# winddori2002/DEX-TTS

Hardware: AMD Instinct MI355X
Metric: mel-frames/s at n_timesteps=50, 80-ch mel (sampler only); RTF (higher is better)
Workload: dtype bf16; 1 GPU; gedex_b1: gedex_lj B=1/GPU T=512 n_timesteps=50 (BASELINE.json configs[1]); global_batch=1, frames=512, hipgraph=False, parallelism=1 GPU

## Files before the change

dex_tts_amd/csrc/dex_api.hip:

```cpp
#include <hip/hip_runtime.h>
#include <cstdlib>

#include <cmath>
#include <cstdarg>
#include <atomic>
#include <cstdio>
#include <mutex>
#include <cstring>
#include <map>
#include <unordered_map>
#include <string_view>
#include <string>
#include <vector>

#include "../../include/dex_amd.h"
#include "kernels.h"
#include "weight_store.h"

using namespace dex;

namespace dex {
namespace {
const char* const KNOB_NAMES[] = {
    "DEX_CONV_STREAM", "DEX_CONV_PP", "DEX_CONV_SKIP_DEAD", "DEX_H_BF16", "DEX_ATTN_SEPARATE", "DEX_ATTN_Q64", "DEX_ATTN_Q64_TAIL", "DEX_ATTN_Q64_HALF", "DEX_DIT_XCDS", "DEX_ATTN_GENERIC", "DEX_RES2", "DEX_LP_INTER", "DEX_DIT_CHAIN",
    "DEX_DIT_CLUSTER", "DEX_DIT_CLUSTER_LOCAL", "DEX_ATTN_X_LP", "DEX_RES_X_LP", "DEX_CAT_LP", "DEX_XCD_MAP", "DEX_DEBUG_DROP_HANDOFF", "DEX_PATCH_FUSED",
    "DEX_CONV_DOWN", "DEX_CONVT_UP", "DEX_DEBUG_PLAN",
    "DEX_ATTN_SHARED_W8", "DEX_CONVT_MT", "DEX_CONVT_WGS", "DEX_CONV_DOWN_WGS", "DEX_CONV_REGW", "DEX_CONV_REGW_RES", "DEX_CONV_SMALL_MAX", "DEX_CONV_TH8",
    "DEX_CONV_W8", "DEX_DWCONV_CAP", "DEX_FINAL_CAP", "DEX_FIRST_CAP", "DEX_FIRST_MFMA", "DEX_GEMM_NWALK", "DEX_NWALK_SPLIT", "DEX_NWALK_BM", "DEX_POS_COL", "DEX_POS_COL_MIN",
    "DEX_POS_CT", "DEX_REGW_MIN_TILES", "DEX_REGW_WGS", "DEX_ROWCHAIN64", "DEX_ROWCHAIN64A", "DEX_TIV_CAP", "DEX_TV_CHAIN", "DEX_TIV_FOLD", "DEX_LINATTN_NSUB", "DEX_TV_FOLD", "DEX_OUT2_MIN", "DEX_NWALK_DMA",
    "DEX_LINATTN_HEADWAVES"};
constexpr int N_KNOBS = (int)(sizeof(KNOB_NAMES) / sizeof(KNOB_NAMES[0]));
int knob_parse(const char* e) {
    if (!e) return KNOB_UNSET;
    char* end = nullptr;
    const long v = strtol(e, &end, 10);
    if (end == e) {
        static bool warned = false;
        if (!warned) { warned = true; fprintf(stderr, "libdexamd: ignoring a DEX_* knob whose value '%s' is not an integer\n", e); }
        return KNOB_UNSET;
    }
    return (int)v;
}
struct KnobSnapshot {
    int v[N_KNOBS];
    KnobSnapshot() { for (int i = 0; i < N_KNOBS; ++i) v[i] = knob_parse(getenv(KNOB_NAMES[i])); }
};
thread_local const KnobSnapshot* t_knobs = nullptr;
struct WsplitScope {
    bool prev;
    explicit WsplitScope(bool on) : prev(g_lp_wsplit) { g_lp_wsplit = on; }
    ~WsplitScope() { g_lp_wsplit = prev; }
};
struct KnobScope {
    const KnobSnapshot* prev;
    explicit KnobScope(const KnobSnapshot* k) : prev(t_knobs) { t_knobs = k; }
    ~KnobScope() { t_knobs = prev; }
};
}
static int knob_index(const char* name) {
    static const std::unordered_map<std::string_view, int> idx = [] {
        std::unordered_map<std::string_view, int> m;
        for (int i = 0; i < N_KNOBS; ++i) m.emplace(KNOB_NAMES[i], i);
        return m;
    }();
    const auto it = idx.find(std::string_view(name));
    return it == idx.end() ? -1 : it->second;
}
int knob(const char* name) {
    if (t_knobs) {
        const int i = knob_index(name);
        if (i >= 0) return t_knobs->v[i];
    }
    return knob_parse(getenv(name));
}
}
static_assert(PREC_FP32 == DEX_PREC_FP32 && PREC_BF16 == DEX_PREC_BF16 && PREC_FP16 == DEX_PREC_FP16 && PREC_FP16X2 == DEX_PREC_FP16X2, "kernels.h mirrors DexPrecision");

namespace {
void xcd_map_probe();

struct TD { float* p; int ld; int coff; int C; int lp = 0; };

struct ResW { const float *w1, *b1, *g1, *be1, *w2, *b2, *g2, *be2, *wr, *br, *mlp_w, *mlp_b; int cin, cout; };
// ... 865 lines not shown
    }

    bool lp_inter_cur = false;
    bool cat_lp = false;
    IGemmP final_gemm(int mask_ws, float* out, int ldo, int ocoff) {
        const DexConfig& c = x->cfg;
        const int hid = c.dit_hidden, mid = mid_dim(c);
        const bool fuse_lnf = x->lp() && ln_fusable(hid);
        const int s2c = c.dit_stride * c.dit_stride * mid;
        IGemmP fl = base_gemm(fuse_lnf ? P.tok : P.xn, hid, 0, P.Hf, P.Wt, hid, x->fl_w, s2c, x->fl_b, out, ldo, ocoff);
        if (fuse_lnf) { fl.ln_shift = P.fin_mod; fl.ln_scale = P.fin_mod + hid; fl.ln_step_stride = 2L * hid; }
        { auto it = x->frag_of().find(x->fl_w); fl.Wfrag = (it != x->frag_of().end()) ? it->second : nullptr; }
        fl.unpatch_s = c.dit_stride; fl.unpatch_C = mid; fl.OHf = P.Hm; fl.OWf = P.Wm;
        fl.c_bstride = (long)P.Hm * P.Wm * ldo;
        fl.outmask = mask; fl.outmask_ws = mask_ws;
        return fl;
    }
    bool linattn_fused(int C) const { return x->lp() && (C == 64 || C == 128) && linattn_fused_supported(C); }
    void linattn(const LinW& w, const StageBuf& s, const TD& X, float* out, int ldo, int ocoff, const LinKvCtxP* tail = nullptr, bool out_lp = false,
                 void* out2_lp = nullptr, int ldo2 = 0, int ocoff2 = 0) {
        const long npix = s.npix; const int B = P.d.B;
        if (linattn_fused(X.C)) {
            int nsub = 1;
            while (nsub < 4 && (npix + 128 * nsub - 1) / (128 * nsub) * B > 192) nsub *= 2;
            {
                const int ncu = device_cus();
                const long slots = (long)(X.C == 64 ? 2 : 1) * ncu;
                if ((npix + 127) / 128 * B >= 2 * slots) {
                    long best = -1;
                    for (int n = 1; n <= 8; ++n) {
                        const long wgs = (npix + 128L * n - 1) / (128L * n) * B;
                        const long cost = (wgs + slots - 1) / slots * n;
                        if (best < 0 || cost <= best) { best = cost; nsub = n; }
                    }
                }
                const int forced = knob_or("DEX_LINATTN_NSUB", 0);
                if (forced > 0) nsub = forced;
            }
            const int nblk = (int)((npix + 128L * nsub - 1) / (128L * nsub));
            LinKvCtxP k{};
            if (tail) k = *tail;
            k.X = X.p; k.ldx = X.ld; k.x_coff = X.coff; k.xb = npix * X.ld; k.npix = (int)npix; k.C = X.C; k.Wkv = w.wkv_lp[x->lpi()];
            k.wkv_lo_off = x->lpi() == 2 ? 384L * X.C : 0;
            k.nsub = nsub; k.nblk = nblk; k.part_m = s.pm; k.part_s = s.ps; k.part_c = s.pc; k.B = B;
            k.headwaves = knob_or("DEX_LINATTN_HEADWAVES", (long)nblk * B <= device_cus() ? 1 : 0) != 0 ? 1 : 0;
            const bool xlp = k.H2 && k.Xout && lp_inter_cur && linattn_out2_lp_out_supported((int)npix, B) && !knob_off("DEX_ATTN_X_LP");
            k.xout_lp = xlp ? 1 : 0;
            run("linattn_kvctx", 2.0 * npix * B * (256.0 * X.C + 128 * 32), (tail ? (tail->h2_bf16 ? 10.0 : 12.0) - (xlp ? 2.0 : 0.0) : 4.0) * npix * X.C * B, [&] { launch_linattn_kvctx(k, x->precision, st); });
            LinMergeP mg{s.pm, s.ps, s.pc, nblk, w.wout_raw, w.g, X.C, s.mbf, B};
            run("linattn_merge", 2.0 * 128 * 32 * X.C * B, 4.0 * nblk * 4 * 1088 * B, [&] { launch_linattn_merge(mg, x->precision, st); });
            LinOut2P o{X.p, X.ld, X.coff, npix * X.ld, (int)npix, X.C, w.wq_frag[x->lpi()], s.mbf, w.bias_eff, out, ldo, ocoff, npix * ldo, B, out_lp ? 1 : 0,
                       out2_lp, ldo2, ocoff2, npix * ldo2, xlp ? 1 : 0};
            o.wq_lo_off = x->lpi() == 2 ? 128L * X.C : 0;
            run("linattn_out", 4.0 * npix * B * 128.0 * X.C, ((out_lp ? 6.0 : 8.0) - (xlp ? 2.0 : 0.0) + (out2_lp ? 2.0 : 0.0)) * npix * X.C * B, [&] { launch_linattn_out2(o, x->precision, st); });
            return;
        }
        IGemmP g = base_gemm(X.p, X.ld, X.coff, s.H, s.W, X.C, w.wqkv, 384, nullptr, s.qkv, 384, 0);
        gemm("linattn_qkv", g);
        LinAttnCtxP cp{s.qkv, 384, npix * 384, (int)npix, 4, LA_CHUNK, s.nchunks, s.pm, s.ps, s.pc, B};
        run("linattn_ctx", 2.0 * npix * 128 * 32 * B, 4.0 * npix * 384 * B, [&] { launch_linattn_ctx(cp, st); });
        LinAttnCombineP cb{s.pm, s.ps, s.pc, s.nchunks, 4, w.wout_raw, w.g, w.C, s.weff, B};
        run("linattn_combine", 2.0 * 128 * 32 * w.C * B, 4.0 * s.nchunks * 4 * 1100 * B, [&] { launch_linattn_combine(cb, st); });
        IGemmP o = base_gemm(s.qkv, 384, 0, s.H, s.W, 128, s.weff, w.C, w.bias_eff, out, ldo, ocoff);
        o.w_bstride = 128L * w.C;
        o.res = X.p; o.ldres = X.ld; o.res_coff = X.coff; o.res_bstride = npix * X.ld;
        gemm("linattn_out", o);
    }

    void dit(const TD& X, bool mask_input, int mask_ws, float* out, int ldo, int ocoff, const float* in_aff = nullptr) {
        const DexConfig& c = x->cfg;
        const int B = P.d.B, hid = c.dit_hidden, mid = mid_dim(c), N = P.N, mh = mlp_hidden(c);
        DwConvP dw{};
        dw.X = X.p + X.coff; dw.ldx = X.ld; dw.xb = (long)P.Hm * P.Wm * X.ld; dw.Hi = P.Hm; dw.Wi = P.Wm; dw.C = mid;
        dw.k = c.dit_patch; dw.s = c.dit_stride; dw.pad = c.dit_patch / 2; dw.Wd = x->pe_dw; dw.bd = x->pe_db;
        dw.mask = mask_input ? mask : nullptr; dw.mask_ws = mask_ws; dw.mask_bstride = P.d.T;
        dw.Y = P.pe0; dw.Hf = P.Hf; dw.Wt = P.Wt; dw.B = B; dw.aff = in_aff;
        auto pw_lp = x->lp_of().find(x->pe_pw);
        if (patch_fused()) {
            run("patch_embed", 2.0 * B * N * mid * (c.dit_patch * c.dit_patch + hid), 4.0 * B * (P.Hm * P.Wm * mid + N * hid),
                [&] { launch_patch_embed_fused(dw, pw_lp->second, x->pe_pb, P.emb, hid, x->precision, st); });
        } else {
            run("patch_dwconv_silu", 2.0 * B * N * mid * c.dit_patch * c.dit_patch, 4.0 * B * (P.Hm * P.Wm + N) * mid, [&] { launch_dwconv_silu(dw, st); });
            IGemmP pe = base_gemm(P.pe0, mid, 0, P.Hf, P.Wt, mid, x->pe_pw, hid, x->pe_pb, P.emb, hid, 0);
            gemm("patch_pointwise", pe);
        }
        const int G = c.dit_conv_pos_groups, kp = c.dit_conv_pos, cg = hid / G;
        int nsplit = POS_SPLIT, pcg = 0, pcgp = 0;
        if (x->lp() && x->pos_wfrag[x->lpi()]) {
            PosConvP pcd{P.emb, x->pos_wfrag[x->lpi()], P.pos_part, P.Hf, P.Wt, hid, G, B};
            run("pos_conv", 2.0 * B * N * (double)kp * kp * cg * hid, 8.0 * B * N * hid + 2.0 * kp * kp * cg * hid, [&] { launch_pos_conv_direct(pcd, x->precision, st); });
            nsplit = 1;
        } else {
            const int cgp = (cg % 32) ? 64 : cg;
            const float* src = P.emb;
            if (cgp != cg) {
                run("pos_group_pad", 0, 8.0 * B * N * hid, [&] { launch_group_pad(P.emb, P.emb_pad, (long)B * N, G, cg, cgp, st); });
                src = P.emb_pad;
            }
            IGemmP pc = base_gemm(src, G * cgp, 0, P.Hf, P.Wt, cgp, x->pos_w, cgp, nullptr, P.pos_part, G * cgp, 0);
            pc.KH = kp; pc.KW = kp; pc.off_h = -(kp / 2); pc.off_w = -(kp / 2); pc.K = kp * kp * cgp;
            pc.groups = G; pc.w_gstride = (long)kp * kp * cgp * cgp; pc.ksplit = POS_SPLIT; pc.c_sstride = (long)B * N * G * cgp;
            if (cgp != cg) pc.Wbf = nullptr;
            gemm("pos_conv", pc);
            pcg = cgp != cg ? cg : 0; pcgp = cgp;
        }
        PosFinishP pf{P.pos_part, nsplit, (long)B * N * (pcg ? G * pcgp : hid), x->pos_b, P.emb, x->freq_pos, P.tok, P.Hf, P.Wt, hid, B, pcg, pcgp};
// ... 813 lines not shown
```

dex_tts_amd/csrc/kernels.h:

```cpp
#pragma once
#include <hip/hip_runtime.h>
#include <stdint.h>

namespace dex {

constexpr int KNOB_UNSET = -2147483647 - 1;
int knob(const char* name);
inline int knob_or(const char* name, int dflt) { const int v = knob(name); return v == KNOB_UNSET ? dflt : v; }
inline bool knob_off(const char* name) { return knob(name) == 0; }
inline bool knob_set(const char* name) { return knob(name) != KNOB_UNSET; }
inline int device_cus() {
    static const int n = [] { int dev = 0, v = 0; (void)hipGetDevice(&dev); (void)hipDeviceGetAttribute(&v, hipDeviceAttributeMultiprocessorCount, dev); return v > 0 ? v : 256; }();
    return n;
}

constexpr int GN_SLOTS = 32;
typedef long long gnfix_t;

extern thread_local const char* g_last_symbol;

constexpr int PREC_FP32 = 0, PREC_BF16 = 1, PREC_FP16 = 2, PREC_FP16X2 = 3;
inline bool prec_wsplit(int precision) { return precision == PREC_FP16X2; }
extern thread_local bool g_lp_wsplit;
inline bool prec_is_lp(int precision) { return precision != PREC_FP32; }
// ... 98 lines not shown
};
void launch_gn_apply(const GnApplyP& p, hipStream_t st);

struct FinalP {
    const float* X; long xb; int npix, W, C, groups; const gnfix_t* stats; const float* gamma; const float* beta;
    const float* mask; long mask_bstride;
    const float* wfc; const float* bfc;
    const float* xcur;
    float* denoised;
    float* xnext;
    const float* scal; int scal_stride; int step;
    float* zero_ptr; long zero_n;
    int B;
    int mode; const float* htab; float* dbuf; const float* xhat;
    int x_bf16;
    const int* poison;
};
void launch_final(const FinalP& p, hipStream_t st);
void launch_churn_tables(const float* sigmas, int n, float S_churn, float S_min, float S_max, float S_noise,
                         float* t_hat, float* h, float* ncoef, hipStream_t st);
void launch_add_noise(float* x, const float* noise, const float* ncoef_i, long n, hipStream_t st);
void launch_heun_expand(const float* t_hat, const float* h, int n, float* sig, float* hout, hipStream_t st);

struct LinAttnCtxP { const float* qkv; int ld; long bstride; int n; int heads; int chunk; int nchunks;
                     float* part_m; float* part_s; float* part_c; int B; };
void launch_linattn_ctx(const LinAttnCtxP& p, hipStream_t st);
struct LinAttnCombineP { const float* part_m; const float* part_s; const float* part_c; int nchunks; int heads;
                         const float* Wout;
                         const float* g;
                         int C; float* Weff;
                         int B; };
void launch_linattn_combine(const LinAttnCombineP& p, hipStream_t st);

struct LinKvCtxP { const float* X; int ldx; int x_coff; long xb; int npix; int C; const void* Wkv; int nsub; int nblk;
                   float* part_m; float* part_s; float* part_c; int B;
                   const float* H2; const gnfix_t* gn_stats; const float* gamma; const float* beta;
                   const float* res; int ldres; long resb; int res_under_mask;
                   const float* mask; int mask_ws; long mask_bstride; int W; float* Xout;
                   int h2_bf16;
                   int res_lp;
                   int xout_lp;     long wkv_lo_off = 0;
                   int headwaves = 0;
                   long long* dbg = nullptr;
};
void launch_linattn_kvctx(const LinKvCtxP& p, int precision, hipStream_t st);
struct LinMergeP { const float* part_m; const float* part_s; const float* part_c; int nblk;
                   const float* Wout; const float* g; int C; void* W2; int B; };
void launch_linattn_merge(const LinMergeP& p, int precision, hipStream_t st);
struct LinOut2P { const float* X; int ldx; int x_coff; long xb; int npix; int C; const void* Wq; const void* W2;
                  const float* bias; float* Y; int ldy; int y_coff; long yb; int B;
                  int y_lp;
                  void* Y2; int ldy2; int y2_coff; long y2b;
                  int x_lp;     long wq_lo_off = 0;
                  };
void launch_linattn_out2(const LinOut2P& p, int precision, hipStream_t st);
bool linattn_out2_lp_out_supported(int npix, int B);
bool linattn_fused_supported(int C);

struct DwConvP { const float* X; int ldx; long xb; int Hi, Wi, C; int k, s, pad; const float* Wd; const float* bd;
                 const float* mask; int mask_ws; long mask_bstride;
                 float* Y; int Hf, Wt; int B;
                 const float* aff = nullptr; };
void launch_dwconv_silu(const DwConvP& p, hipStream_t st);
bool patch_embed_fused_supported(int k, int C, int hid, long ntok);
void launch_patch_embed_fused(const DwConvP& p, const void* Wb, const float* bias, float* emb, int hid, int precision, hipStream_t st);

struct PosConvP { const float* X; const void* Wf; float* Y; int Hf, Wt, hid, G, B;
                  int ncol; };
bool pos_conv_direct_supported(int hid, int groups, int kernel, int Hf);
void launch_pos_conv_direct(const PosConvP& p, int precision, hipStream_t st);
struct PosFinishP { const float* part; int nsplit; long split_stride; const float* bias; const float* emb;
                    const float* freq_pos; float* tok; int Hf, Wt, D; int B;
                    int cg, cg_pad; };
void launch_pos_finish(const PosFinishP& p, hipStream_t st);
void launch_group_pad(const float* src, float* dst, long rows, int G, int cg, int cg_pad, hipStream_t st);

struct LnModP { const float* X; float* Y; int rows_per_batch; int D; const float* shift; const float* scale;
                long step_stride; int step; int B; };
void launch_ln_mod(const LnModP& p, hipStream_t st);

struct DitChainP { const float* O; int ksplit; long o_sstride; const float* ml; int heads; int rows_per_batch;
                   float* X; const void *Wp, *W1, *W2, *Wq; const float *bp, *b1, *b2, *bq;
                   const float* ada;
                   const float *next_shift, *next_scale; long next_step_stride;
                   void *Qh, *Kh, *Vt; int Npad; float qscale;
                   const void *Qin, *Kin, *Vin;
                   int qkv_only;
                   int attn_inline;
                   int step; int M; int B; long long* dbg;
                   float* xslab; unsigned* xflag; unsigned epoch; int* xerr;
                   int o_lp;
                   int xcd_map;
                   int xlocal;
                   int xdrop;
                   int tail_row0 = 0, tail_ks = 0;
                   int xcds = 8; };
constexpr int DIT_CLUSTER = 4;
constexpr size_t DIT_CLUSTER_SLAB_FLOATS = 2 * DIT_CLUSTER * (32 * 256 + 256);
constexpr size_t DIT_CLUSTER_FLAG_WORDS = 2 * DIT_CLUSTER;
bool dit_rowchain64_form(int rows_per_batch, int B, int attn_inline);
bool dit_rowchain_cluster_form(int rows_per_batch, int B);
bool dit_rowchain_cluster_local_fits(int rows_per_batch, int B);
int dit_rowchain_cluster_xcds(int rows_per_batch, int B);
bool dit_rowchain_supported(int hidden, int mlp_hidden);
struct AttnDirectP { const void *Qh, *Kh, *Vt; int N, Npad, B; float* O; long o_sstride; float* ml; int ksplit; long long* dbg;
                     int o_lp;
// ... 144 lines not shown
```

dex_tts_amd/csrc/linattn_fused.hip:

```cpp
#include "kernels.h"
#include "lp_util.h"
#include "kernels_lp.h"

namespace dex {
namespace DEX_LP_NS {

typedef float f32x16 __attribute__((ext_vector_type(16)));
typedef unsigned short u16;
union LFrag { uint4 u; lp8 v; };
constexpr float LOG2E_F = 1.4426950408889634f;


#ifdef DEX_TIMING
#define KSTAMP_DECL long long tk[8] = {0, 0, 0, 0, 0, 0, 0, 0}; const long long tk0 = __builtin_readcyclecounter(); long long tlast = tk0;
#define KSTAMP(k) do { const long long now_ = __builtin_readcyclecounter(); tk[k] += now_ - tlast; tlast = now_; } while (0)
#define KSTAMP_STORE(n)                                                                                               \
    if (p.dbg && threadIdx.x == 0) {                                                                                  \
        long long* d_ = p.dbg + ((long)blockIdx.y * gridDim.x + blockIdx.x) * 8;                                      \
        for (int k_ = 0; k_ < (n); ++k_) d_[k_] = tk[k_];                                                             \
        d_[7] = __builtin_readcyclecounter() - tk0;                                                                   \
    }
#else
#define KSTAMP_DECL
#define KSTAMP(k) do {} while (0)
// ... 340 lines not shown
    }
    __syncthreads();
    float* mS = reinterpret_cast<float*>(smem_la);
    float* mm = mS + 4 * 4 * 32 * 33;
    float* ms = mm + 4 * 4 * 32;
#pragma unroll
    for (int h = 0; h < 4; ++h) {
        const float st = s_run[h] + __shfl_xor(s_run[h], 32);
        float* dst = mS + ((wave * 4 + h) * 32 + i) * 33;
#pragma unroll
        for (int r = 0; r < 16; ++r) dst[(r & 3) + 8 * (r >> 2) + 4 * hh] = ctxT[h][r];
        if (hh == 0) { mm[(wave * 4 + h) * 32 + i] = m_run[h]; ms[(wave * 4 + h) * 32 + i] = st; }
    }
    __syncthreads();
    KSTAMP(5);
    for (int idx = tid; idx < 4 * 1024; idx += 256) {
        const int h = idx >> 10, d = (idx >> 5) & 31, e = idx & 31;
        float M = -INFINITY;
#pragma unroll
        for (int w = 0; w < 4; ++w) M = fmaxf(M, mm[(w * 4 + h) * 32 + d]);
        float acc = 0.f, s = 0.f;
#pragma unroll
        for (int w = 0; w < 4; ++w) {
            const float mw = mm[(w * 4 + h) * 32 + d];
            const float f = (mw == -INFINITY) ? 0.f : __expf(mw - M);
            acc = fmaf(f, mS[((w * 4 + h) * 32 + d) * 33 + e], acc);
            s = fmaf(f, ms[(w * 4 + h) * 32 + d], s);
        }
        const long pidx = ((long)b * 4 + h) * p.nblk + blk;
        p.part_c[pidx * 1024 + d * 32 + e] = acc;
        if (e == 0) { p.part_m[pidx * 32 + d] = M; p.part_s[pidx * 32 + d] = s; }
    }
    KSTAMP(6);
    KSTAMP_STORE(7)
}

template <int C, bool PRO, int FL = -1>
__global__ __launch_bounds__(1024) void linattn_kvctx_hw_kernel(const LinKvCtxP p) {
    constexpr int LDW = C + 8, KS = C / 16, KQ = KS / 4;
#ifdef DEX_LP_WSPLIT
    constexpr int NWI = 2;
#else
    constexpr int NWI = 1;
#endif
    extern __shared__ __attribute__((aligned(16))) u16 smem_la[];
    u16* Ws = smem_la;
    u16* Xs = smem_la + NWI * 256 * LDW;
    KSTAMP_DECL
    const int tid = threadIdx.x, lane = tid & 63, wave = tid >> 6;
    const int hd = wave & 3, slot = wave >> 2;
    const int i = lane & 31, hh = lane >> 5;
    const int blk = blockIdx.x, b = blockIdx.y;
    const u16* Wg = reinterpret_cast<const u16*>(p.Wkv);
    {
        uint4 wr[C / 32];
#pragma unroll
        for (int j = 0; j < C / 32; ++j) {
            const int it = tid + 1024 * j;
            wr[j] = *reinterpret_cast<const uint4*>(Wg + (long)(it / (C / 8)) * C + (it % (C / 8)) * 8);
        }
#pragma unroll
        for (int j = 0; j < C / 32; ++j) {
            const int it = tid + 1024 * j;
            *reinterpret_cast<uint4*>(Ws + (it / (C / 8)) * LDW + (it % (C / 8)) * 8) = wr[j];
        }
#ifdef DEX_LP_WSPLIT
#pragma unroll
        for (int j = 0; j < C / 32; ++j) {
            const int it = tid + 1024 * j;
            wr[j] = *reinterpret_cast<const uint4*>(Wg + p.wkv_lo_off + (long)(it / (C / 8)) * C + (it % (C / 8)) * 8);
        }
#pragma unroll
        for (int j = 0; j < C / 32; ++j) {
            const int it = tid + 1024 * j;
            *reinterpret_cast<uint4*>(Ws + 256 * LDW + (it / (C / 8)) * LDW + (it % (C / 8)) * 8) = wr[j];
        }
#endif
    }
    const float* X = PRO ? p.H2 + (long)b * p.npix * C : p.X + (long)b * p.xb + p.x_coff;
    const int ldx = PRO ? C : p.ldx;
    const float* R = (PRO && p.res) ? p.res + (long)b * p.resb : nullptr;
    const float* mrow = PRO ? p.mask + (long)b * p.mask_bstride : nullptr;
    const int px_base = (blk * 4 + slot) * p.nsub * 32;
    const int ch0 = hd * KQ * 16 + hh * 8;

    f32x16 ctxT;
    float m_run = -INFINITY, s_run = 0.f;
#pragma unroll
    for (int r = 0; r < 16; ++r) ctxT[r] = 0.f;
    float4 xa[KQ], xc[KQ], ra[PRO ? KQ : 1], rc[PRO ? KQ : 1];
    float mkv = 1.f;
    float ga_pre = 0.f, be_pre = 0.f;
    if constexpr (PRO) { if (tid < C) { ga_pre = p.gamma[tid]; be_pre = p.beta[tid]; } }
    const bool hb = FL >= 0 ? (FL & 1) != 0 : (PRO && p.h2_bf16 != 0);
    const bool rlp = FL >= 0 ? (FL & 2) != 0 : (PRO && p.res_lp != 0);
    const bool xlp = FL >= 0 ? (FL & 4) != 0 : (p.xout_lp != 0);
    const unsigned short* Rh = (PRO && p.res) ? reinterpret_cast<const unsigned short*>(p.res) + (long)b * p.resb : nullptr;
    const unsigned short* Xh = PRO ? reinterpret_cast<const unsigned short*>(p.H2) + (long)b * p.npix * C : nullptr;
    auto load_rows = [&](int px0) {
        const int pxr = min(px0 + i, p.npix - 1);
        if (hb) {
#pragma unroll
            for (int ks = 0; ks < KQ; ++ks) { xa[ks] = *reinterpret_cast<const float4*>(Xh + (long)pxr * C + ch0 + ks * 16); xc[ks] = xa[ks]; }
        } else {
            const float* xr = X + (long)pxr * ldx + ch0;
#pragma unroll
            for (int ks = 0; ks < KQ; ++ks) {
                xa[ks] = *reinterpret_cast<const float4*>(xr + ks * 16);
                xc[ks] = *reinterpret_cast<const float4*>(xr + ks * 16 + 4);
            }
        }
        if constexpr (PRO) {
            if (R) {
                if (rlp) {
#pragma unroll
                    for (int ks = 0; ks < KQ; ++ks) { ra[ks] = *reinterpret_cast<const float4*>(Rh + (long)pxr * p.ldres + ch0 + ks * 16); rc[ks] = ra[ks]; }
                } else {
                    const float* rr = R + (long)pxr * p.ldres + ch0;
#pragma unroll
                    for (int ks = 0; ks < KQ; ++ks) {
                        ra[ks] = *reinterpret_cast<const float4*>(rr + ks * 16);
                        rc[ks] = *reinterpret_cast<const float4*>(rr + ks * 16 + 4);
                    }
                }
            }
            mkv = mrow[(pxr % p.W) * p.mask_ws];
        }
    };
    load_rows(px_base);
    KSTAMP(0);
    __shared__ float smean[8], srstd[8];
    __shared__ __attribute__((aligned(16))) float gsc_s[PRO ? C : 4], gsh_s[PRO ? C : 4];
    if constexpr (PRO) {
        if (tid < 256) {
            const int g = tid / GN_SLOTS;
            const longlong2 sv = *reinterpret_cast<const longlong2*>(p.gn_stats + (((long)b * 8 + g) * GN_SLOTS + (tid % GN_SLOTS)) * 2);
            long long s1 = sv.x, s2 = sv.y;
            gn_slots_reduce<GN_SLOTS>(s1, s2);
            if ((tid % GN_SLOTS) == 0) gn_moments(s1, s2, 1e-5, smean[g], srstd[g]);
        }
    }
    __syncthreads();
    if constexpr (PRO) {
        if (tid < C) {
            const float ga = ga_pre * srstd[tid / (C / 8)];
            gsc_s[tid] = ga;
            gsh_s[tid] = be_pre - smean[tid / (C / 8)] * ga;
        }
        __syncthreads();
    }
    KSTAMP(1);
    constexpr bool SEED = C == 128 || (FL >= 0 && (FL & 2) != 0);
    for (int sub = 0; sub < p.nsub; ++sub) {
        const int px0 = px_base + sub * 32;
        const bool act = px0 < p.npix;
        u16* xs = Xs + ((slot * 2 + (sub & 1)) * 32 + i) * LDW;
        if (act) {
            if constexpr (PRO) {
                const bool under = FL >= 0 ? (FL & 8) != 0 : (p.res_under_mask != 0);
                const bool live = px0 + i < p.npix;
                const long orow = (long)b * p.npix + min(px0 + i, p.npix - 1);
#pragma unroll
                for (int ks = 0; ks < KQ; ++ks)
                    kv_prologue8(p, xa[ks], xc[ks], ra[ks], rc[ks], gsc_s, gsh_s, ch0 + ks * 16, hb, rlp, R != nullptr, under, xlp, mkv, live, orow);
            }
#pragma unroll
            for (int ks = 0; ks < KQ; ++ks)
                *reinterpret_cast<uint4*>(xs + ch0 + ks * 16) =
                    make_uint4(pack2_lp(xa[ks].x, xa[ks].y), pack2_lp(xa[ks].z, xa[ks].w), pack2_lp(xc[ks].x, xc[ks].y), pack2_lp(xc[ks].z, xc[ks].w));
            if (sub + 1 < p.nsub) load_rows(px0 + 32);
        }
        KSTAMP(2);
        __syncthreads();
        KSTAMP(3);
        if (!act) continue;
        LFrag af[KS];
#pragma unroll
        for (int ks = 0; ks < KS; ++ks) af[ks].u = *reinterpret_cast<const uint4*>(xs + ks * 16 + hh * 8);
        f32x16 kseed;
#pragma unroll
        for (int r = 0; r < 16; ++r) kseed[r] = (SEED && px0 + (r & 3) + 8 * (r >> 2) + 4 * hh >= p.npix) ? -INFINITY : 0.f;
        kv_head_step<C, SEED, (C == 128 ? 4 : 0)>(Ws, hd, i, hh, af, kseed, px0, p.npix, ctxT, m_run, s_run);
        KSTAMP(4);
    }
    __syncthreads();
    float* mS = reinterpret_cast<float*>(smem_la);
    float* mm = mS + 4 * 4 * 32 * 33;
    float* ms = mm + 4 * 4 * 32;
    {
        const float st = s_run + __shfl_xor(s_run, 32);
        float* dst = mS + ((slot * 4 + hd) * 32 + i) * 33;
#pragma unroll
        for (int r = 0; r < 16; ++r) dst[(r & 3) + 8 * (r >> 2) + 4 * hh] = ctxT[r];
        if (hh == 0) { mm[(slot * 4 + hd) * 32 + i] = m_run; ms[(slot * 4 + hd) * 32 + i] = st; }
    }
    __syncthreads();
    KSTAMP(5);
    for (int idx = tid; idx < 4 * 1024; idx += 1024) {
        const int h = idx >> 10, d = (idx >> 5) & 31, e = idx & 31;
        float M = -INFINITY;
#pragma unroll
        for (int w = 0; w < 4; ++w) M = fmaxf(M, mm[(w * 4 + h) * 32 + d]);
// ... 121 lines not shown
__global__ __launch_bounds__(256) void linattn_merge_kernel(const LinMergeP p) {
    __shared__ float redm[8], reda[8][32], reds[8], cvec[32];
    const int tid = threadIdx.x, h = blockIdx.x, b = blockIdx.y, d = blockIdx.z;
    const int C = p.C;
    float4 wo[8];
    if (tid < C) {
#pragma unroll
        for (int j = 0; j < 8; ++j) wo[j] = *reinterpret_cast<const float4*>(p.Wout + (long)tid * 128 + h * 32 + j * 4);
    }
    const float g = p.g[0];
    const long pbase = ((long)b * 4 + h) * p.nblk;
    const int e = tid & 31, pl = tid >> 5;
    float m = -INFINITY, acc = 0.f, s = 0.f;
    const int per_lane = (p.nblk + 7) / 8;
    if (per_lane <= 8) merge_fold<8>(p, pbase, d, e, pl, m, acc, s);
    else if (per_lane <= 16) merge_fold<16>(p, pbase, d, e, pl, m, acc, s);
    else merge_fold<24>(p, pbase, d, e, pl, m, acc, s);
    if (e == 0) { redm[pl] = m; reds[pl] = s; }
    reda[pl][e] = acc;
    __syncthreads();
    if (pl == 0) {
        float M = redm[0];
#pragma unroll
        for (int k = 1; k < 8; ++k) M = fmaxf(M, redm[k]);
        float a = 0.f, ss = 0.f;
#pragma unroll
        for (int k = 0; k < 8; ++k) {
            const float w = (redm[k] == -INFINITY) ? 0.f : __expf(redm[k] - M);
            a = fmaf(w, reda[k][e], a); ss = fmaf(w, reds[k], ss);
        }
        cvec[e] = a / ss;
    }
    __syncthreads();
    if (tid < C) {
        float a = 0.f;
#pragma unroll
        for (int j = 0; j < 8; ++j) {
            a = fmaf(wo[j].x, cvec[j * 4 + 0], a); a = fmaf(wo[j].y, cvec[j * 4 + 1], a);
            a = fmaf(wo[j].z, cvec[j * 4 + 2], a); a = fmaf(wo[j].w, cvec[j * 4 + 3], a);
        }
        a *= g;
        const int co = tid, hh = (d >> 2) & 1, j = (d & 3) + 4 * ((d >> 3) & 1), ks = 2 * h + (d >> 4);
        const long dst = ((((long)b * (C / 32) + (co >> 5)) * 8 + ks) * 64 + hh * 32 + (co & 31)) * 8 + j;
        reinterpret_cast<u16*>(p.W2)[dst] = (u16)(pack2_lp(a, 0.f) & 0xffffu);
    }
}
void launch_linattn_merge(const LinMergeP& p, hipStream_t st) {
    hipLaunchKernelGGL(linattn_merge_kernel, dim3(4, p.B, 32), dim3(256), 0, st, p);
}

template <int C>
__global__ __launch_bounds__(256) void linattn_out2_direct_kernel(const LinOut2P p) {
    constexpr int KS1 = C / 16, CT = C / 32;
    const int tid = threadIdx.x, lane = tid & 63, wave = tid >> 6;
    const int i = lane & 31, hh = lane >> 5;
    const int b = blockIdx.y;
    const int px0 = (blockIdx.x * 4 + wave) * 32;
    if (px0 >= p.npix) return;
    const float* X = p.X + (long)b * p.xb + p.x_coff;
    const int px = min(px0 + i, p.npix - 1);
    const float* xr = X + (long)px * p.ldx + hh * 8;
    float4 xa[KS1], xc[KS1];
#pragma unroll
    for (int ks = 0; ks < KS1; ++ks) {
        xa[ks] = *reinterpret_cast<const float4*>(xr + ks * 16);
        xc[ks] = *reinterpret_cast<const float4*>(xr + ks * 16 + 4);
    }
    const uint4* w2 = reinterpret_cast<const uint4*>(p.W2) + (long)b * CT * 8 * 64 + lane;
    uint4 w2f[CT][8];
#pragma unroll
    for (int ct = 0; ct < CT; ++ct)
#pragma unroll
        for (int ks = 0; ks < 8; ++ks) w2f[ct][ks] = w2[(ct * 8 + ks) * 64];
    LFrag xf[KS1];
#pragma unroll
    for (int ks = 0; ks < KS1; ++ks) {
        xf[ks].u.x = pack2_lp(xa[ks].x, xa[ks].y); xf[ks].u.y = pack2_lp(xa[ks].z, xa[ks].w);
        xf[ks].u.z = pack2_lp(xc[ks].x, xc[ks].y); xf[ks].u.w = pack2_lp(xc[ks].z, xc[ks].w);
    }
    const uint4* wq = reinterpret_cast<const uint4*>(p.Wq) + lane;
    LFrag qf[8];
#pragma unroll
    for (int t = 0; t < 4; ++t) {
        f32x16 q;
#pragma unroll
        for (int r = 0; r < 16; ++r) q[r] = 0.f;
#pragma unroll
        for (int ks = 0; ks < KS1; ++ks) {
            LFrag af; af.u = wq[(t * KS1 + ks) * 64];
            q = DEX_MFMA_LP(af.v, xf[ks].v, q, 0, 0, 0);
#ifdef DEX_LP_WSPLIT
            LFrag al; al.u = wq[(t * KS1 + ks) * 64 + p.wq_lo_off / 8];
            q = DEX_MFMA_LP(al.v, xf[ks].v, q, 0, 0, 0);
#endif
        }
#pragma unroll
        for (int k2 = 0; k2 < 2; ++k2) {
            qf[t * 2 + k2].u.x = pack2_lp(q[8 * k2 + 0], q[8 * k2 + 1]); qf[t * 2 + k2].u.y = pack2_lp(q[8 * k2 + 2], q[8 * k2 + 3]);
            qf[t * 2 + k2].u.z = pack2_lp(q[8 * k2 + 4], q[8 * k2 + 5]); qf[t * 2 + k2].u.w = pack2_lp(q[8 * k2 + 6], q[8 * k2 + 7]);
        }
    }
    float* Y = p.Y + (long)b * p.yb + p.y_coff;
    const bool ok = px0 + i < p.npix;
#pragma unroll
    for (int ct = 0; ct < CT; ++ct) {
        f32x16 y;
#pragma unroll
        for (int r = 0; r < 16; ++r) y[r] = 0.f;
        float4 res[4], bia[4];
#pragma unroll
        for (int g4 = 0; g4 < 4; ++g4) {
            const int co = ct * 32 + 8 * g4 + 4 * hh;
            res[g4] = *reinterpret_cast<const float4*>(X + (long)px * p.ldx + co);
            bia[g4] = *reinterpret_cast<const float4*>(p.bias + co);
        }
#pragma unroll
        for (int ks = 0; ks < 8; ++ks) {
            LFrag af; af.u = w2f[ct][ks];
            y = DEX_MFMA_LP(af.v, qf[ks].v, y, 0, 0, 0);
        }
        if (ok) {
#pragma unroll
            for (int g4 = 0; g4 < 4; ++g4) {
                const int co = ct * 32 + 8 * g4 + 4 * hh;
                float4 o;
                o.x = y[g4 * 4 + 0] + res[g4].x + bia[g4].x; o.y = y[g4 * 4 + 1] + res[g4].y + bia[g4].y;
                o.z = y[g4 * 4 + 2] + res[g4].z + bia[g4].z; o.w = y[g4 * 4 + 3] + res[g4].w + bia[g4].w;
                *reinterpret_cast<float4*>(Y + (long)(px0 + i) * p.ldy + co) = o;
            }
        }
    }
}
template <int C>
__global__ __launch_bounds__(256) __attribute__((amdgpu_waves_per_eu(2, C == 64 ? 4 : 2))) void linattn_out2_kernel(const LinOut2P p) {
    constexpr int KS1 = C / 16, CT = C / 32;
    constexpr int LDX = C + 4;
    constexpr int NCH = 32 * C / 4 / 64;
    extern __shared__ __attribute__((aligned(16))) float smem_o2[];
    const int tid = threadIdx.x, lane = tid & 63, wave = tid >> 6;
    const int i = lane & 31, hh = lane >> 5;
    const int b = blockIdx.y;
    const int px0 = (blockIdx.x * 4 + wave) * 32;
    if (px0 >= p.npix) return;
    float* xs = smem_o2 + wave * 32 * LDX;
    const float* X = p.X + (long)b * p.xb + p.x_coff;
    float4 xin[NCH];
    const bool xlp = p.x_lp != 0;
    if (xlp) {
        const u16* Xh = reinterpret_cast<const u16*>(p.X) + (long)b * p.xb + p.x_coff;
#pragma unroll
        for (int k = 0; k < NCH / 2; ++k) {
            const int c = lane + 64 * k, px = c / (C / 8), ch = (c % (C / 8)) * 8;
            xin[k] = *reinterpret_cast<const float4*>(Xh + (long)min(px0 + px, p.npix - 1) * p.ldx + ch);
        }
    } else {
#pragma unroll
        for (int k = 0; k < NCH; ++k) {
            const int c = lane + 64 * k, px = c / (C / 4), ch = (c % (C / 4)) * 4;
            xin[k] = *reinterpret_cast<const float4*>(X + (long)min(px0 + px, p.npix - 1) * p.ldx + ch);
        }
    }
    const uint4* w2 = reinterpret_cast<const uint4*>(p.W2) + (long)b * CT * 8 * 64 + lane;
    uint4 w2f[CT][8];
#pragma unroll
    for (int ct = 0; ct < CT; ++ct)
#pragma unroll
        for (int ks = 0; ks < 8; ++ks) w2f[ct][ks] = w2[(ct * 8 + ks) * 64];
    if (xlp) {
#pragma unroll
        for (int k = 0; k < NCH / 2; ++k) {
            const int c = lane + 64 * k, px = c / (C / 8), ch = (c % (C / 8)) * 8;
            const unsigned u0 = __float_as_uint(xin[k].x), u1 = __float_as_uint(xin[k].y), u2 = __float_as_uint(xin[k].z), u3 = __float_as_uint(xin[k].w);
            *reinterpret_cast<float4*>(xs + px * LDX + ch) = make_float4(lp_lo(u0), lp_hi(u0), lp_lo(u1), lp_hi(u1));
            *reinterpret_cast<float4*>(xs + px * LDX + ch + 4) = make_float4(lp_lo(u2), lp_hi(u2), lp_lo(u3), lp_hi(u3));
        }
    } else {
#pragma unroll
        for (int k = 0; k < NCH; ++k) {
            const int c = lane + 64 * k, px = c / (C / 4), ch = (c % (C / 4)) * 4;
            *reinterpret_cast<float4*>(xs + px * LDX + ch) = xin[k];
        }
    }
    __builtin_amdgcn_wave_barrier();
    LFrag xf[KS1];
// ... 32 lines not shown
#pragma unroll
        for (int r = 0; r < 16; ++r) y[r] = 0.f;
#pragma unroll
        for (int ks = 0; ks < 8; ++ks) {
            LFrag af; af.u = w2f[ct][ks];
            y = DEX_MFMA_LP(af.v, qf[ks].v, y, 0, 0, 0);
        }
#pragma unroll
        for (int g4 = 0; g4 < 4; ++g4) {
            const int co = ct * 32 + 8 * g4 + 4 * hh;
            float* slot = xs + i * LDX + co;
            const float4 res = *reinterpret_cast<const float4*>(slot);
            const float4 bia = *reinterpret_cast<const float4*>(p.bias + co);
            float4 o;
            o.x = y[g4 * 4 + 0] + res.x + bia.x; o.y = y[g4 * 4 + 1] + res.y + bia.y;
            o.z = y[g4 * 4 + 2] + res.z + bia.z; o.w = y[g4 * 4 + 3] + res.w + bia.w;
            *reinterpret_cast<float4*>(slot) = o;
        }
    }
    __builtin_amdgcn_wave_barrier();
    float* Y = p.Y + (long)b * p.yb + p.y_coff;
#pragma unroll
    for (int k = 0; k < NCH; ++k) {
        const int c = lane + 64 * k, px = c / (C / 4), ch = (c % (C / 4)) * 4;
        const float4 o = *reinterpret_cast<const float4*>(xs + px * LDX + ch);
        if (px0 + px < p.npix) {
            if (p.y_lp) {
                u16* yh = reinterpret_cast<u16*>(p.Y) + (long)b * p.yb + p.y_coff + (long)(px0 + px) * p.ldy + ch;
                *reinterpret_cast<uint2*>(yh) = make_uint2(pack2_lp(o.x, o.y), pack2_lp(o.z, o.w));
            } else *reinterpret_cast<float4*>(Y + (long)(px0 + px) * p.ldy + ch) = o;
            if (p.Y2) {
                u16* y2 = reinterpret_cast<u16*>(p.Y2) + (long)b * p.y2b + p.y2_coff + (long)(px0 + px) * p.ldy2 + ch;
                *reinterpret_cast<uint2*>(y2) = make_uint2(pack2_lp(o.x, o.y), pack2_lp(o.z, o.w));
            }
        }
    }
}
bool linattn_fused_supported(int C) {
#if defined(DEX_LP_WSPLIT) && !defined(DEX_WS_HAVE_LINATTN)
    return false;
#endif
    return C == 64 || C == 128;
}
static long out2_min_wgs() { return knob_or("DEX_OUT2_MIN", 256); }
bool linattn_out2_lp_out_supported(int npix, int B) { return (long)((npix + 127) / 128) * B >= out2_min_wgs(); }
void launch_linattn_out2(const LinOut2P& p, hipStream_t st) {
    dim3 grid((p.npix + 127) / 128, p.B);
    const size_t lds = (size_t)4 * 32 * (p.C + 4) * sizeof(float);
    static bool attr = false;
    if (!attr) {
        hipFuncSetAttribute(reinterpret_cast<const void*>(&linattn_out2_kernel<128>), hipFuncAttributeMaxDynamicSharedMemorySize, (int)((size_t)4 * 32 * 132 * sizeof(float)));
        attr = true;
    }
    if ((long)grid.x * p.B < out2_min_wgs()) {
        if (p.C == 64) hipLaunchKernelGGL(linattn_out2_direct_kernel<64>, grid, dim3(256), 0, st, p);
        else hipLaunchKernelGGL(linattn_out2_direct_kernel<128>, grid, dim3(256), 0, st, p);
        return;
    }
    if (p.C == 64) hipLaunchKernelGGL(linattn_out2_kernel<64>, grid, dim3(256), lds, st, p);
    else hipLaunchKernelGGL(linattn_out2_kernel<128>, grid, dim3(256), lds, st, p);
}

}
}
```

Measured before the change: 27000 mel-frames/s.

## Add head-wave split linattn out kernel for small grids; prefetch GN stats

Adds a linattn_out2_hw kernel in which each 256-thread block handles 32 pixels instead of 128. The four waves split the first GEMM's K dimension and exchange bf16 fragments through LDS, so small-batch cases launch four times as many workgroups and fill more CUs. It is selected by default when the grid is too small for the LDS-staged path and no low-precision I/O is in use. Separately, the kvctx kernel now issues its GN-stat, gamma and beta loads earlier to hide their latency, and uses lds_barrier instead of __syncthreads. The cost is extra LDS barriers and redundant weight loads per pixel, plus some timing-stamp instrumentation.

```diff
diff --git a/dex_tts_amd/csrc/dex_api.hip b/dex_tts_amd/csrc/dex_api.hip
--- a/dex_tts_amd/csrc/dex_api.hip
+++ b/dex_tts_amd/csrc/dex_api.hip
@@ -28,7 +28,7 @@
     "DEX_ATTN_SHARED_W8", "DEX_CONVT_MT", "DEX_CONVT_WGS", "DEX_CONV_DOWN_WGS", "DEX_CONV_REGW", "DEX_CONV_REGW_RES", "DEX_CONV_SMALL_MAX", "DEX_CONV_TH8",
     "DEX_CONV_W8", "DEX_DWCONV_CAP", "DEX_FINAL_CAP", "DEX_FIRST_CAP", "DEX_FIRST_MFMA", "DEX_GEMM_NWALK", "DEX_NWALK_SPLIT", "DEX_NWALK_BM", "DEX_POS_COL", "DEX_POS_COL_MIN",
     "DEX_POS_CT", "DEX_REGW_MIN_TILES", "DEX_REGW_WGS", "DEX_ROWCHAIN64", "DEX_ROWCHAIN64A", "DEX_TIV_CAP", "DEX_TV_CHAIN", "DEX_TIV_FOLD", "DEX_LINATTN_NSUB", "DEX_TV_FOLD", "DEX_OUT2_MIN", "DEX_NWALK_DMA",
-    "DEX_LINATTN_HEADWAVES"};
+    "DEX_LINATTN_HEADWAVES", "DEX_LINATTN_OUT2_HW"};
 constexpr int N_KNOBS = (int)(sizeof(KNOB_NAMES) / sizeof(KNOB_NAMES[0]));
 int knob_parse(const char* e) {
     if (!e) return KNOB_UNSET;
@@ -1000,6 +1000,7 @@
             LinOut2P o{X.p, X.ld, X.coff, npix * X.ld, (int)npix, X.C, w.wq_frag[x->lpi()], s.mbf, w.bias_eff, out, ldo, ocoff, npix * ldo, B, out_lp ? 1 : 0,
                        out2_lp, ldo2, ocoff2, npix * ldo2, xlp ? 1 : 0};
             o.wq_lo_off = x->lpi() == 2 ? 128L * X.C : 0;
+            o.hw = knob_or("DEX_LINATTN_OUT2_HW", linattn_out2_lp_out_supported((int)npix, B) ? 0 : 1) != 0 ? 1 : 0;
             run("linattn_out", 4.0 * npix * B * 128.0 * X.C, ((out_lp ? 6.0 : 8.0) - (xlp ? 2.0 : 0.0) + (out2_lp ? 2.0 : 0.0)) * npix * X.C * B, [&] { launch_linattn_out2(o, x->precision, st); });
             return;
         }
diff --git a/dex_tts_amd/csrc/kernels.h b/dex_tts_amd/csrc/kernels.h
--- a/dex_tts_amd/csrc/kernels.h
+++ b/dex_tts_amd/csrc/kernels.h
@@ -174,6 +174,8 @@
                   int y_lp;
                   void* Y2; int ldy2; int y2_coff; long y2b;
                   int x_lp;     long wq_lo_off = 0;
+                  int hw = 0;
+                  long long* dbg = nullptr;
                   };
 void launch_linattn_out2(const LinOut2P& p, int precision, hipStream_t st);
 bool linattn_out2_lp_out_supported(int npix, int B);
diff --git a/dex_tts_amd/csrc/linattn_fused.hip b/dex_tts_amd/csrc/linattn_fused.hip
--- a/dex_tts_amd/csrc/linattn_fused.hip
+++ b/dex_tts_amd/csrc/linattn_fused.hip
@@ -416,6 +416,12 @@
     const int i = lane & 31, hh = lane >> 5;
     const int blk = blockIdx.x, b = blockIdx.y;
     const u16* Wg = reinterpret_cast<const u16*>(p.Wkv);
+    uint4 sv = make_uint4(0u, 0u, 0u, 0u);
+    float ga_pre = 0.f, be_pre = 0.f;
+    if constexpr (PRO) {
+        if (tid < 8 * GN_SLOTS) sv = *reinterpret_cast<const uint4*>(p.gn_stats + (((long)b * 8 + tid / GN_SLOTS) * GN_SLOTS + (tid % GN_SLOTS)) * 2);
+        if (tid < C) { ga_pre = p.gamma[tid]; be_pre = p.beta[tid]; }
+    }
     {
         uint4 wr[C / 32];
 #pragma unroll
@@ -454,8 +460,6 @@
     for (int r = 0; r < 16; ++r) ctxT[r] = 0.f;
     float4 xa[KQ], xc[KQ], ra[PRO ? KQ : 1], rc[PRO ? KQ : 1];
     float mkv = 1.f;
-    float ga_pre = 0.f, be_pre = 0.f;
-    if constexpr (PRO) { if (tid < C) { ga_pre = p.gamma[tid]; be_pre = p.beta[tid]; } }
     const bool hb = FL >= 0 ? (FL & 1) != 0 : (PRO && p.h2_bf16 != 0);
     const bool rlp = FL >= 0 ? (FL & 2) != 0 : (PRO && p.res_lp != 0);
     const bool xlp = FL >= 0 ? (FL & 4) != 0 : (p.xout_lp != 0);
@@ -496,22 +500,22 @@
     __shared__ float smean[8], srstd[8];
     __shared__ __attribute__((aligned(16))) float gsc_s[PRO ? C : 4], gsh_s[PRO ? C : 4];
     if constexpr (PRO) {
-        if (tid < 256) {
+        if (tid < 8 * GN_SLOTS) {
             const int g = tid / GN_SLOTS;
-            const longlong2 sv = *reinterpret_cast<const longlong2*>(p.gn_stats + (((long)b * 8 + g) * GN_SLOTS + (tid % GN_SLOTS)) * 2);
-            long long s1 = sv.x, s2 = sv.y;
+            long long s1 = (long long)(((unsigned long long)mov_pinned(sv.y) << 32) | mov_pinned(sv.x));
+            long long s2 = (long long)(((unsigned long long)mov_pinned(sv.w) << 32) | mov_pinned(sv.z));
             gn_slots_reduce<GN_SLOTS>(s1, s2);
             if ((tid % GN_SLOTS) == 0) gn_moments(s1, s2, 1e-5, smean[g], srstd[g]);
         }
     }
-    __syncthreads();
+    lds_barrier();
     if constexpr (PRO) {
         if (tid < C) {
             const float ga = ga_pre * srstd[tid / (C / 8)];
             gsc_s[tid] = ga;
             gsh_s[tid] = be_pre - smean[tid / (C / 8)] * ga;
         }
-        __syncthreads();
+        lds_barrier();
     }
     KSTAMP(1);
     constexpr bool SEED = C == 128 || (FL >= 0 && (FL & 2) != 0);
@@ -739,6 +743,7 @@
 template <int C>
 __global__ __launch_bounds__(256) void linattn_out2_direct_kernel(const LinOut2P p) {
     constexpr int KS1 = C / 16, CT = C / 32;
+    KSTAMP_DECL
     const int tid = threadIdx.x, lane = tid & 63, wave = tid >> 6;
     const int i = lane & 31, hh = lane >> 5;
     const int b = blockIdx.y;
@@ -759,6 +764,7 @@
     for (int ct = 0; ct < CT; ++ct)
 #pragma unroll
         for (int ks = 0; ks < 8; ++ks) w2f[ct][ks] = w2[(ct * 8 + ks) * 64];
+    KSTAMP(0);
     LFrag xf[KS1];
 #pragma unroll
     for (int ks = 0; ks < KS1; ++ks) {
@@ -787,6 +793,7 @@
             qf[t * 2 + k2].u.z = pack2_lp(q[8 * k2 + 4], q[8 * k2 + 5]); qf[t * 2 + k2].u.w = pack2_lp(q[8 * k2 + 6], q[8 * k2 + 7]);
         }
     }
+    KSTAMP(2);
     float* Y = p.Y + (long)b * p.yb + p.y_coff;
     const bool ok = px0 + i < p.npix;
 #pragma unroll
@@ -806,6 +813,7 @@
             LFrag af; af.u = w2f[ct][ks];
             y = DEX_MFMA_LP(af.v, qf[ks].v, y, 0, 0, 0);
         }
+        KSTAMP(4);
         if (ok) {
 #pragma unroll
             for (int g4 = 0; g4 < 4; ++g4) {
@@ -816,7 +824,134 @@
                 *reinterpret_cast<float4*>(Y + (long)(px0 + i) * p.ldy + co) = o;
             }
         }
-    }
+        KSTAMP(5);
+    }
+    KSTAMP_STORE(7)
+}
+
+template <int C>
+__global__ __launch_bounds__(256) void linattn_out2_hw_kernel(const LinOut2P p) {
+    constexpr int KS1 = C / 16, CT = C / 32, KQ = KS1 / 4;
+    __shared__ uint4 xs[KS1][64], qs[8][64];
+    KSTAMP_DECL
+    const int tid = threadIdx.x, lane = tid & 63;
+    const int t = __builtin_amdgcn_readfirstlane(tid >> 6);
+    const int i = lane & 31, hh = lane >> 5;
+    const int b = blockIdx.y;
+    const int px0 = blockIdx.x * 32;
+    if (px0 >= p.npix) return;
+    const float* X = p.X + (long)b * p.xb + p.x_coff;
+    const int px = min(px0 + i, p.npix - 1);
+    float4 xa[KQ], xc[KQ];
+    const float* xr = X + (long)px * p.ldx + hh * 8;
+#pragma unroll
+    for (int k = 0; k < KQ; ++k) {
+        const int ks = t * KQ + k;
+        xa[k] = *reinterpret_cast<const float4*>(xr + ks * 16);
+        xc[k] = *reinterpret_cast<const float4*>(xr + ks * 16 + 4);
+    }
+    const uint4* wq = reinterpret_cast<const uint4*>(p.Wq) + lane;
+    uint4 wqf[KS1];
+#ifdef DEX_LP_WSPLIT
+    uint4 wql[KS1];
+#endif
+#pragma unroll
+    for (int ks = 0; ks < KS1; ++ks) {
+        wqf[ks] = wq[(t * KS1 + ks) * 64];
+#ifdef DEX_LP_WSPLIT
+        wql[ks] = wq[(t * KS1 + ks) * 64 + p.wq_lo_off / 8];
+#endif
+    }
+    const bool g2 = t < CT;
+    const int ct = g2 ? t : 0;
+    const uint4* w2 = reinterpret_cast<const uint4*>(p.W2) + (long)b * CT * 8 * 64 + lane;
+    uint4 w2f[8];
+    float4 res[4], bia[4];
+    if (g2) {
+#pragma unroll
+        for (int ks = 0; ks < 8; ++ks) w2f[ks] = w2[(ct * 8 + ks) * 64];
+        if constexpr (C != 128) {
+#pragma unroll
+            for (int g4 = 0; g4 < 4; ++g4) res[g4] = *reinterpret_cast<const float4*>(X + (long)px * p.ldx + ct * 32 + 8 * g4 + 4 * hh);
+        }
+        const float4* bt = reinterpret_cast<const float4*>(p.bias + ct * 32);
+        const unsigned hm = 0u - (unsigned)hh;
+#pragma unroll
+        for (int g4 = 0; g4 < 4; ++g4) {
+            const float4 b0 = bt[2 * g4], b1 = bt[2 * g4 + 1];
+            bia[g4] = make_float4(__uint_as_float((__float_as_uint(b1.x) & hm) | (__float_as_uint(b0.x) & ~hm)),
+                                  __uint_as_float((__float_as_uint(b1.y) & hm) | (__float_as_uint(b0.y) & ~hm)),
+                                  __uint_as_float((__float_as_uint(b1.z) & hm) | (__float_as_uint(b0.z) & ~hm)),
+                                  __uint_as_float((__float_as_uint(b1.w) & hm) | (__float_as_uint(b0.w) & ~hm)));
+        }
+    }
+    KSTAMP(0);
+#pragma unroll
+    for (int k = 0; k < KQ; ++k) {
+        LFrag f;
+        f.u.x = pack2_lp(xa[k].x, xa[k].y); f.u.y = pack2_lp(xa[k].z, xa[k].w);
+        f.u.z = pack2_lp(xc[k].x, xc[k].y); f.u.w = pack2_lp(xc[k].z, xc[k].w);
+        xs[t * KQ + k][lane] = f.u;
+    }
+    if constexpr (C == 128) {
+#pragma unroll
+        for (int k = 0; k < 2; ++k) {
+            const float4 snd = hh ? xa[k] : xc[k];
+            float4 rcv;
+            rcv.x = __shfl_xor(snd.x, 32); rcv.y = __shfl_xor(snd.y, 32); rcv.z = __shfl_xor(snd.z, 32); rcv.w = __shfl_xor(snd.w, 32);
+            res[2 * k] = hh ? rcv : xa[k];
+            res[2 * k + 1] = hh ? xc[k] : rcv;
+        }
+    }
+    lds_barrier();
+    KSTAMP(1);
+    {
+        f32x16 q;
+#pragma unroll
+        for (int r = 0; r < 16; ++r) q[r] = 0.f;
+#pragma unroll
+        for (int ks = 0; ks < KS1; ++ks) {
+            LFrag af, xf; af.u = wqf[ks]; xf.u = xs[ks][lane];
+            q = DEX_MFMA_LP(af.v, xf.v, q, 0, 0, 0);
+#ifdef DEX_LP_WSPLIT
+            LFrag al; al.u = wql[ks];
+            q = DEX_MFMA_LP(al.v, xf.v, q, 0, 0, 0);
+#endif
+        }
+#pragma unroll
+        for (int k2 = 0; k2 < 2; ++k2) {
+            LFrag f;
+            f.u.x = pack2_lp(q[8 * k2 + 0], q[8 * k2 + 1]); f.u.y = pack2_lp(q[8 * k2 + 2], q[8 * k2 + 3]);
+            f.u.z = pack2_lp(q[8 * k2 + 4], q[8 * k2 + 5]); f.u.w = pack2_lp(q[8 * k2 + 6], q[8 * k2 + 7]);
+            qs[t * 2 + k2][lane] = f.u;
+        }
+    }
+    KSTAMP(2);
+    lds_barrier();
+    KSTAMP(3);
+    if (!g2) return;
+    f32x16 y;
+#pragma unroll
+    for (int r = 0; r < 16; ++r) y[r] = 0.f;
+#pragma unroll
+    for (int ks = 0; ks < 8; ++ks) {
+        LFrag af, qf; af.u = w2f[ks]; qf.u = qs[ks][lane];
+        y = DEX_MFMA_LP(af.v, qf.v, y, 0, 0, 0);
+    }
+    KSTAMP(4);
+    float* Y = p.Y + (long)b * p.yb + p.y_coff;
+    if (px0 + i < p.npix) {
+#pragma unroll
+        for (int g4 = 0; g4 < 4; ++g4) {
+            const int co = ct * 32 + 8 * g4 + 4 * hh;
+            float4 o;
+            o.x = y[g4 * 4 + 0] + res[g4].x + bia[g4].x; o.y = y[g4 * 4 + 1] + res[g4].y + bia[g4].y;
+            o.z = y[g4 * 4 + 2] + res[g4].z + bia[g4].z; o.w = y[g4 * 4 + 3] + res[g4].w + bia[g4].w;
+            *reinterpret_cast<float4*>(Y + (long)(px0 + i) * p.ldy + co) = o;
+        }
+    }
+    KSTAMP(5);
+    KSTAMP_STORE(7)
 }
 template <int C>
 __global__ __launch_bounds__(256) __attribute__((amdgpu_waves_per_eu(2, C == 64 ? 4 : 2))) void linattn_out2_kernel(const LinOut2P p) {
@@ -955,6 +1090,14 @@
         hipFuncSetAttribute(reinterpret_cast<const void*>(&linattn_out2_kernel<128>), hipFuncAttributeMaxDynamicSharedMemorySize, (int)((size_t)4 * 32 * 132 * sizeof(float)));
         attr = true;
     }
+    const bool lp_io = p.x_lp || p.y_lp || p.Y2;
+    if (p.hw && !lp_io) {
+        g_last_symbol = "linattn_out2_hw_kernel";
+        const dim3 g1((p.npix + 31) / 32, p.B);
+        if (p.C == 64) hipLaunchKernelGGL(linattn_out2_hw_kernel<64>, g1, dim3(256), 0, st, p);
+        else hipLaunchKernelGGL(linattn_out2_hw_kernel<128>, g1, dim3(256), 0, st, p);
+        return;
+    }
     if ((long)grid.x * p.B < out2_min_wgs()) {
         if (p.C == 64) hipLaunchKernelGGL(linattn_out2_direct_kernel<64>, grid, dim3(256), 0, st, p);
         else hipLaunchKernelGGL(linattn_out2_direct_kernel<128>, grid, dim3(256), 0, st, p);
```

Measured after the change: 27480 mel-frames/s, median of 6. +1.8%, better.
